# lhn0323/BEVFUSION-3D_object_detection

Hardware: AMD Instinct MI355X
Metric: nuScenes frames/sec (6-cam+LiDAR BEVFusion fwd+bwd) (higher is better)
Workload: dtype bf16; 1 GPU; full: BEVFusion camera+LiDAR (ResNet-50, LSS 6x256x704, hard voxelize 40k pts, sparse encoder, ConvFuser, SECOND/SECONDFPN, TransFusion head + Hungarian targets + focal/L1/gaussian-focal losses) fwd + bwd + clip + AdamW, bf16 autocast, fp32 index paths; global_batch=4, points_per_frame=40000, parallelism=independent frames per rank, execution=eager launches on 2 HIP queues (camera / BEV chain, LiDAR branch), view_transform_conv_dtype=bf16, head_fp32_conv=three bf16 products per multiply, fp32 accumulation (2^-16 relative per product), dense_weight_gradients=one grouped launch per tile shape at the end of the backward pass, backward_pass_thread=caller, trainable_params=37361053

## Files before the change

### bevfusion-3d_object_detection_amd/_lib.py

```python
import ctypes
import os

import torch

_HERE = os.path.dirname(os.path.abspath(__file__))
LIB_PATH = os.path.join(_HERE, "csrc", "libbevfusion_hip.so")

_c_int = ctypes.c_int
_c_vp = ctypes.c_void_p
_c_sz = ctypes.c_size_t

SIGNATURES = {
    "bfhip_abi_version": (_c_int, []),
    "bfhip_last_error": (ctypes.c_char_p, []),
    "bfhip_profile_enable": (None, [_c_int]),
    "bfhip_profile_read": (_c_int, [_c_int, _c_vp, _c_vp, _c_int]),
    "bfhip_bev_pool_fwd": (_c_int, [_c_vp] * 5 + [_c_int] * 7 + [_c_vp, _c_vp]),
    "bfhip_bev_pool_bwd": (_c_int, [_c_vp] * 5 + [_c_int] * 8 + [_c_vp, _c_vp]),
    "bfhip_dynamic_voxelize": (_c_int, [_c_vp, _c_vp, _c_int, _c_int, _c_vp, _c_vp, _c_vp]),
    "bfhip_hard_voxelize_workspace_bytes": (_c_sz, [_c_int, _c_int, _c_int]),
    "bfhip_hard_voxelize": (_c_int, [_c_vp, _c_int, _c_int, _c_vp, _c_vp, _c_vp, _c_vp, _c_vp,
                                     _c_int, _c_int, _c_vp, _c_sz, _c_vp, _c_vp]),
    "bfhip_bev_plan_workspace_bytes": (_c_sz, [ctypes.c_longlong, ctypes.c_longlong]),
    "bfhip_bev_plan": (_c_int, [_c_vp] * 7 + [_c_int] * 4 + [_c_vp] * 3 + [_c_vp] * 11 + [_c_int, _c_vp, _c_sz, _c_vp]),
# ... 80 lines not shown
    "bfhip_conv2d_wt_segment_bytes": (_c_int, []),
    "bfhip_conv2d_weight_transpose_batched": (_c_int, [_c_vp, _c_int, ctypes.c_longlong, _c_vp]),
    "bfhip_conv2d_launch_choice": (_c_int, [_c_int] * 12 + [_c_vp]),
    "bfhip_conv2d_wgrad_choice": (_c_int, [_c_int] * 10 + [_c_vp]),
    "bfhip_conv2d_wgrad_workspace_bytes": (_c_sz, [_c_int] * 7),
    "bfhip_conv2d_wgrad": (_c_int, [_c_vp, _c_int, _c_vp, _c_int, _c_vp] + [_c_int] * 11 + [_c_vp, _c_sz, _c_vp]),
    "bfhip_conv2d_wgrad_group_table_bytes": (_c_sz, [_c_int]),
    "bfhip_conv2d_wgrad_groupable": (_c_int, [_c_int] * 10),
    "bfhip_conv2d_wgrad_group_plan": (_c_int, [_c_vp, _c_int, _c_int, _c_vp, _c_sz, _c_vp]),
    "bfhip_conv2d_wgrad_group_launch": (_c_int, [_c_vp, _c_vp, _c_vp, _c_sz, _c_vp]),
    "bfhip_bn2d_fwd_partials": (_c_int, [_c_vp] * 4 + [ctypes.c_longlong, _c_int, _c_int, ctypes.c_float, ctypes.c_float, _c_int] +
                                [_c_vp] * 4 + [_c_vp, _c_int, _c_vp, _c_vp]),
    "bfhip_bn2d_fwd_partials_mask": (_c_int, [_c_vp] * 4 + [ctypes.c_longlong, _c_int, _c_int, ctypes.c_float, ctypes.c_float, _c_int] +
                                     [_c_vp] * 4 + [_c_vp, _c_int, _c_vp, _c_vp, _c_vp]),
    "bfhip_bn2d_bwd_mask": (_c_int, [_c_vp] * 5 + [ctypes.c_longlong, _c_int, _c_int] + [_c_vp] * 4 + [_c_vp, _c_sz, _c_vp]),
    "bfhip_adamw_segment_bytes": (_c_int, []),
    "bfhip_adamw_chunk_elems": (_c_int, []),
    "bfhip_adamw_step": (_c_int, [_c_vp, _c_vp, _c_vp, _c_int, _c_vp, _c_vp] + [ctypes.c_float] * 6 + [_c_vp]),
    "bfhip_adamw_step_groups": (_c_int, [_c_vp, _c_vp, _c_vp, _c_int, _c_vp, _c_vp, _c_vp, _c_vp, _c_int, ctypes.c_float, _c_vp]),
    "bfhip_query_losses": (_c_int, [_c_vp] * 7 + [_c_int] * 6 + [ctypes.c_float, ctypes.c_float] + [_c_vp] * 4),
    "bfhip_swin_attn_supported": (_c_int, [_c_int] * 7),
    "bfhip_swin_attn_parts": (_c_int, [_c_int] * 4),
    "bfhip_swin_attn_fwd": (_c_int, [_c_vp, ctypes.c_longlong, _c_vp] + [_c_int] * 5 + [ctypes.c_float, _c_vp, _c_vp, _c_vp]),
    "bfhip_swin_attn_bwd": (_c_int, [_c_vp, ctypes.c_longlong, _c_vp, _c_vp, _c_vp, _c_vp] + [_c_int] * 5 +
                            [ctypes.c_float, _c_vp, _c_vp, _c_int, _c_vp]),
    "bfhip_layernorm_supported": (_c_int, [ctypes.c_longlong, _c_int, _c_int, _c_int]),
    "bfhip_layernorm_parts": (_c_int, [ctypes.c_longlong, _c_int]),
    "bfhip_layernorm_fwd": (_c_int, [_c_vp, _c_vp, _c_vp, ctypes.c_longlong, _c_vp, _c_vp, ctypes.c_longlong, _c_int, ctypes.c_float] +
                            [_c_int] * 3 + [_c_vp] * 4),
    "bfhip_layernorm_bwd": (_c_int, [_c_vp] * 6 + [ctypes.c_longlong, ctypes.c_longlong] + [_c_int] * 4 + [_c_vp] * 3 + [_c_int] +
# ... 125 lines not shown
```

### bevfusion-3d_object_detection_amd/csrc/bn2d.hip

```cpp
#include <algorithm>
#include <map>
#include <mutex>

#include "common.h"

namespace bfhip {
namespace {

typedef unsigned short bf16_t;

template <typename T> struct Vec;
template <> struct Vec<float> {
  static constexpr int V = 4;
  static __device__ __forceinline__ void load(const float *p, float *o) {
    float4 v = *(const float4 *)p;
    o[0] = v.x; o[1] = v.y; o[2] = v.z; o[3] = v.w;
  }
  static __device__ __forceinline__ void store(float *p, const float *o) { *(float4 *)p = make_float4(o[0], o[1], o[2], o[3]); }
};
template <> struct Vec<bf16_t> {
  static constexpr int V = 8;
  static __device__ __forceinline__ void load(const bf16_t *p, float *o) {
    uint4 v = *(const uint4 *)p;
    const unsigned w[4] = {v.x, v.y, v.z, v.w};
// ... 99 lines not shown
    for (int g2 = 0; g2 < tr.ng; ++g2) {
      s += ld_agent(&tr.gp[((size_t)g2 * 2 + 0) * C + c]);
      s2 += ld_agent(&tr.gp[((size_t)g2 * 2 + 1) * C + c]);
    }
    fin(c, s, s2);
  }
}

struct FwdFin {
  long long M;
  const int *m_dev;
  int C;
  float eps, momentum;
  const float *gamma, *beta;
  float *stats, *running_mean, *running_var;
  __device__ __forceinline__ void operator()(int c, double s, double s2) const {
    long long Mv = M;
    if (m_dev) { long long mv = *m_dev; Mv = mv < 1 ? 1 : (mv < M ? mv : M); }
    double mean = s / (double)Mv;
    double var = s2 / (double)Mv - mean * mean;
    if (var < 0.0) var = 0.0;
    float invstd = (float)(1.0 / sqrt(var + (double)eps));
    float a = gamma[c] * invstd;
    stats[c] = (float)mean;
    stats[C + c] = invstd;
    stats[2 * C + c] = a;
    stats[3 * C + c] = beta[c] - (float)mean * a;
    if (running_mean) {
      double unbiased = Mv > 1 ? var * (double)Mv / (double)(Mv - 1) : var;
      running_mean[c] = (float)((1.0 - momentum) * running_mean[c] + momentum * mean);
      running_var[c] = (float)((1.0 - momentum) * running_var[c] + momentum * unbiased);
    }
  }
};

struct BwdFin {
  long long M;
  const int *m_dev;
  int C;
  const float *stats;
  float *dgb, *coef;
  __device__ __forceinline__ void operator()(int c, double s, double s2) const {
    long long Mv = M;
    if (m_dev) { long long mv = *m_dev; Mv = mv < 1 ? 1 : (mv < M ? mv : M); }
    const float mean = stats[c], invstd = stats[C + c], a = stats[2 * C + c];
    const float dbeta = (float)s, dgamma = (float)(s2 * (double)invstd);
    dgb[c] = dgamma;
    dgb[C + c] = dbeta;
    const float invM = (float)(1.0 / (double)Mv);
    const float c2 = -a * invstd * dgamma * invM;
    coef[c] = a;
    coef[C + c] = c2;
    coef[2 * C + c] = -a * dbeta * invM - c2 * mean;
  }
};

struct SumFin {
  int C;
  float *out;
  __device__ __forceinline__ void operator()(int c, double s, double) const { out[c] = (float)s; }
};

template <typename T>
__global__ __launch_bounds__(256) void bn2d_stats_kernel(const T *__restrict__ x, long long M, int C, Map mp,
                                                         float *__restrict__ partial, Tree tr, FwdFin fin) {
  constexpr int V = Vec<T>::V;
  __shared__ float sm[2 * 256 * V];
  const int t = threadIdx.x, cv = blockIdx.y * mp.Lb + t % mp.Lb, rl = t / mp.Lb;
// ... 60 lines not shown
  s = 0.0; s2 = 0.0;
  if (t < 8)
#pragma unroll
    for (int g = 0; g < 8; ++g) { s += sm[0][g * 8 + t]; s2 += sm[1][g * 8 + t]; }
}

template <typename Fin>
__global__ __launch_bounds__(kFinThreads) void bn2d_finalize_kernel(const float *__restrict__ partial, int nblk, Fin fin) {
  const int c = blockIdx.x * 8 + (threadIdx.x & 7);
  double s, s2;
  reduce_partials8(partial, nblk, fin.C, c, c < fin.C, s, s2);
  if (threadIdx.x >= 8 || c >= fin.C) return;
  fin(c, s, s2);
}

template <typename T, bool RES, bool RELU>
__global__ __launch_bounds__(256) void bn2d_apply_kernel(const T *__restrict__ x, const T *__restrict__ res,
                                                         const float *__restrict__ stats, long long M, int C, Map mp,
                                                         T *__restrict__ y, unsigned char *__restrict__ relu_mask) {
  constexpr int V = Vec<T>::V;
  const int t = threadIdx.x, cv = blockIdx.y * mp.Lb + t % mp.Lb, rl = t / mp.Lb;
  const bool live = rl < mp.R && cv * V < C;
  if (!live) return;
  float a[V], b[V];
#pragma unroll
  for (int j = 0; j < V; ++j) { a[j] = stats[2 * C + cv * V + j]; b[j] = stats[3 * C + cv * V + j]; }
  const long long r0 = (long long)blockIdx.x * mp.rpb, r1 = r0 + mp.rpb < M ? r0 + mp.rpb : M;
  const size_t col = (size_t)cv * V;
  long long r = r0 + rl;
  for (; r + mp.R < r1; r += 2LL * mp.R) {
    float v[2][V], q[2][V];
#pragma unroll
    for (int u = 0; u < 2; ++u) {
      Vec<T>::load(x + (size_t)(r + (long long)u * mp.R) * C + col, v[u]);
      if (RES) Vec<T>::load(res + (size_t)(r + (long long)u * mp.R) * C + col, q[u]);
    }
#pragma unroll
    for (int u = 0; u < 2; ++u) {
      unsigned bits = 0;
#pragma unroll
      for (int j = 0; j < V; ++j) {
        float o = v[u][j] * a[j] + b[j];
        if (RES) o += q[u][j];
        if (o > 0.f) bits |= 1u << j;
        v[u][j] = (RELU && !(o > 0.f)) ? 0.f : o;
      }
      Vec<T>::store(y + (size_t)(r + (long long)u * mp.R) * C + col, v[u]);
      if (V == 8 && relu_mask) relu_mask[(size_t)(r + (long long)u * mp.R) * (C >> 3) + cv] = (unsigned char)bits;
    }
  }
  for (; r < r1; r += mp.R) {
    float v[V], q[V];
    Vec<T>::load(x + (size_t)r * C + col, v);
    if (RES) Vec<T>::load(res + (size_t)r * C + col, q);
    unsigned bits = 0;
#pragma unroll
    for (int j = 0; j < V; ++j) {
      float o = v[j] * a[j] + b[j];
      if (RES) o += q[j];
      if (o > 0.f) bits |= 1u << j;
      v[j] = (RELU && !(o > 0.f)) ? 0.f : o;
    }
    Vec<T>::store(y + (size_t)r * C + col, v);
    if (V == 8 && relu_mask) relu_mask[(size_t)r * (C >> 3) + cv] = (unsigned char)bits;
  }
}

template <typename T, int MASK>
__device__ __forceinline__ void masked_grad(float *g, const float *xv, const float *yv, const float *a, const float *b) {
  constexpr int V = Vec<T>::V;
  const unsigned bits = MASK == 3 ? __float_as_uint(yv[0]) : 0u;
#pragma unroll
  for (int j = 0; j < V; ++j) {
    if (MASK == 1 && !(xv[j] * a[j] + b[j] > 0.f)) g[j] = 0.f;
    if (MASK == 2 && !(yv[j] > 0.f)) g[j] = 0.f;
    if (MASK == 3 && !((bits >> j) & 1u)) g[j] = 0.f;
  }
}

// ... 41 lines not shown
      float g[V], xv[V], yv[V];
      size_t off = (size_t)r * C + col;
      Vec<T>::load(dy + off, g);
      Vec<T>::load(x + off, xv);
      if (MASK == 2) Vec<T>::load(y + off, yv);
      if (MASK == 3) yv[0] = __uint_as_float(((const unsigned char *)y)[(size_t)r * (C >> 3) + cv]);
      masked_grad<T, MASK>(g, xv, yv, a, b);
#pragma unroll
      for (int j = 0; j < V; ++j) { s0[j] += g[j]; s1[j] += g[j] * (xv[j] - mean[j]); }
    }
  }
  combine_rows<V>(s0, s1, mp.Lb, mp.R, C, partial, sm);
  finish_in_last_block(partial, tr, C, blockIdx.y * mp.Lb * V, mp.Lb * V, fin);
}

template <typename T, int MASK, bool DRES>
__global__ __launch_bounds__(256) void bn2d_bwd_apply_kernel(const T *__restrict__ dy, const T *__restrict__ x,
                                                             const T *__restrict__ y,
                                                             const float *__restrict__ stats,
                                                             const float *__restrict__ coef, long long M, int C,
                                                             Map mp, T *__restrict__ dx, T *__restrict__ dres) {
  constexpr int V = Vec<T>::V;
  const int t = threadIdx.x, cv = blockIdx.y * mp.Lb + t % mp.Lb, rl = t / mp.Lb;
  const bool live = rl < mp.R && cv * V < C;
  if (!live) return;
  float a[V], b[V], c1[V], c2[V], c3[V];
#pragma unroll
  for (int j = 0; j < V; ++j) {
    a[j] = stats[2 * C + cv * V + j];
    b[j] = stats[3 * C + cv * V + j];
    c1[j] = coef[cv * V + j];
    c2[j] = coef[C + cv * V + j];
    c3[j] = coef[2 * C + cv * V + j];
  }
  const long long r0 = (long long)blockIdx.x * mp.rpb, r1 = r0 + mp.rpb < M ? r0 + mp.rpb : M;
  const size_t col = (size_t)cv * V;
  long long r = r0 + rl;
  for (; r + mp.R < r1; r += 2LL * mp.R) {
    float g[2][V], xv[2][V], yv[2][V];
#pragma unroll
    for (int u = 0; u < 2; ++u) {
      size_t off = (size_t)(r + (long long)u * mp.R) * C + col;
      Vec<T>::load(dy + off, g[u]);
      Vec<T>::load(x + off, xv[u]);
      if (MASK == 2) Vec<T>::load(y + off, yv[u]);
      if (MASK == 3) yv[u][0] = __uint_as_float(((const unsigned char *)y)[(size_t)(r + (long long)u * mp.R) * (C >> 3) + cv]);
    }
#pragma unroll
    for (int u = 0; u < 2; ++u) {
      size_t off = (size_t)(r + (long long)u * mp.R) * C + col;
      masked_grad<T, MASK>(g[u], xv[u], yv[u], a, b);
      if (DRES) Vec<T>::store(dres + off, g[u]);
#pragma unroll
      for (int j = 0; j < V; ++j) xv[u][j] = c1[j] * g[u][j] + c2[j] * xv[u][j] + c3[j];
      Vec<T>::store(dx + off, xv[u]);
    }
  }
  for (; r < r1; r += mp.R) {
    float g[V], xv[V], yv[V];
    size_t off = (size_t)r * C + col;
    Vec<T>::load(dy + off, g);
    Vec<T>::load(x + off, xv);
    if (MASK == 2) Vec<T>::load(y + off, yv);
    if (MASK == 3) yv[0] = __uint_as_float(((const unsigned char *)y)[(size_t)r * (C >> 3) + cv]);
    masked_grad<T, MASK>(g, xv, yv, a, b);
    if (DRES) Vec<T>::store(dres + off, g);
#pragma unroll
    for (int j = 0; j < V; ++j) xv[j] = c1[j] * g[j] + c2[j] * xv[j] + c3[j];
    Vec<T>::store(dx + off, xv);
  }
}

inline int elem_size(int dtype) { return dtype == 1 ? 2 : 4; }

inline bool shape_ok(long long M, int C, int dtype) {
  const int V = 16 / elem_size(dtype);
  return M > 0 && C >= V && C % V == 0 && C <= 65536;
}

inline Map make_map(long long M, int C, int dtype, dim3 *grid) {
  const int es = elem_size(dtype), V = 16 / es, L = C / V;
  Map mp;
  mp.Lb = L < 32 ? L : 32;
  mp.R = 256 / mp.Lb;
  const int CT = (L + mp.Lb - 1) / mp.Lb;
  long long S = 1024;
  S = std::min(S, (M + 4LL * mp.R - 1) / (4LL * mp.R));
  S = std::min(S, (long long)std::max(1, 2048 / CT));
  S = std::min(S, std::max(1LL, M * es / 128));
  S = std::max(S, 1LL);
  long long rpb = ((M + S - 1) / S + mp.R - 1) / mp.R * mp.R;
  S = (M + rpb - 1) / rpb;
  mp.rpb = (int)rpb;
  *grid = dim3((unsigned)S, (unsigned)CT);
  return mp;
}

template <typename T>
int run_fwd(const void *x, const void *res, const float *stats, long long M, int C, Map mp, dim3 grid, int relu, void *y,
            hipStream_t s, unsigned char *relu_mask = nullptr) {
#define BFHIP_BN2D_APPLY(RES, RELU)                                                                             \
  hipLaunchKernelGGL((bn2d_apply_kernel<T, RES, RELU>), grid, dim3(256), 0, s, (const T *)x, (const T *)res, \
                     stats, M, C, mp, (T *)y, (RES && RELU) ? relu_mask : (unsigned char *)nullptr)
  if (res) { if (relu) BFHIP_BN2D_APPLY(true, true); else BFHIP_BN2D_APPLY(true, false); }
  else { if (relu) BFHIP_BN2D_APPLY(false, true); else BFHIP_BN2D_APPLY(false, false); }
#undef BFHIP_BN2D_APPLY
  return 0;
}

template <typename T, int MASK>
void run_bwd(const void *dy, const void *x, const void *y, const float *stats, long long M, int C, Map mp, dim3 grid,
             float *partial, float *coef, Tree tr, BwdFin fin, void *dx, void *dres, hipStream_t s) {
  hipLaunchKernelGGL((bn2d_bwd_reduce_kernel<T, MASK>), grid, dim3(256), 0, s, (const T *)dy, (const T *)x,
                     (const T *)y, stats, M, C, mp, partial, tr, fin);
  if (!tr.cnt) hipLaunchKernelGGL(bn2d_finalize_kernel<BwdFin>, dim3(ceil_div(C, 8)), dim3(kFinThreads), 0, s, partial, tr.nblk, fin);
  if (dres)
    hipLaunchKernelGGL((bn2d_bwd_apply_kernel<T, MASK, true>), grid, dim3(256), 0, s, (const T *)dy, (const T *)x,
                       (const T *)y, stats, coef, M, C, mp, (T *)dx, (T *)dres);
  else
    hipLaunchKernelGGL((bn2d_bwd_apply_kernel<T, MASK, false>), grid, dim3(256), 0, s, (const T *)dy,
                       (const T *)x, (const T *)y, stats, coef, M, C, mp, (T *)dx, (T *)nullptr);
}

constexpr int kSlabInts = 16384;
constexpr int kSlabs = 32;

inline bool fold_enabled() {
  static const bool on = [] { const char *e = env_str("BFHIP_BN2D_FOLD"); return e && e[0] == '1'; }();
  return on;
}

int *arrival_counters(hipStream_t stream) {
  static std::mutex mu;
  static std::map<int, int *> pool;
  static std::map<std::pair<int, hipStream_t>, int> slot;
  static std::map<int, int> used;
  int dev = 0;
  if (hipGetDevice(&dev) != hipSuccess) return nullptr;
  std::lock_guard<std::mutex> lock(mu);
  auto it = pool.find(dev);
  if (it == pool.end()) {
    int *p = nullptr;
    const size_t bytes = (size_t)kSlabs * kSlabInts * sizeof(int);
    if (hipMalloc((void **)&p, bytes) != hipSuccess || hipMemset(p, 0, bytes) != hipSuccess) {
      set_error("bn2d: cannot allocate the arrival counters (first call on a device must be outside a stream capture)");
// ... 2 lines not shown
    it = pool.emplace(dev, p).first;
  }
  auto key = std::make_pair(dev, stream);
  auto st = slot.find(key);
  if (st == slot.end()) {
    if (used[dev] >= kSlabs) { set_error("bn2d: more than %d streams per device in use", kSlabs); return nullptr; }
    st = slot.emplace(key, used[dev]++).first;
  }
  return it->second + (size_t)st->second * kSlabInts;
}

struct Plan {
  Map mp;
  dim3 grid;
  int nblk, ng;
  float *partial, *coef;
  double *gp;
};

inline size_t plan_bytes(long long M, int C, int dtype, Plan *pl, void *workspace) {
  pl->mp = make_map(M, C, dtype, &pl->grid);
  pl->nblk = (int)pl->grid.x;
  pl->ng = (pl->nblk + kGroup - 1) / kGroup;
  size_t off = 0;
  pl->partial = (float *)((char *)workspace + off); off += align_up((size_t)pl->nblk * 2 * C * sizeof(float), 256);
  pl->coef = (float *)((char *)workspace + off); off += align_up((size_t)3 * C * sizeof(float), 256);
  pl->gp = (double *)((char *)workspace + off); off += align_up((size_t)pl->ng * 2 * C * sizeof(double), 256);
  return off;
}

}
}

using namespace bfhip;

BFHIP_EXPORT int bfhip_bn2d_supported(long long M, int C, int dtype) {
  return (dtype == 0 || dtype == 1) && shape_ok(M, C, dtype) ? 1 : 0;
}

BFHIP_EXPORT size_t bfhip_bn2d_workspace_bytes(long long M, int C, int dtype) {
  if (!bfhip_bn2d_supported(M, C, dtype)) return 0;
  Plan pl;
  return plan_bytes(M, C, dtype, &pl, nullptr);
}

BFHIP_EXPORT int bfhip_colsum(const void *x, long long M, int C, int dtype, float *out, void *workspace, size_t workspace_bytes,
                              void *stream_) {
  hipStream_t s = (hipStream_t)stream_;
  BFHIP_REQUIRE(bfhip_bn2d_supported(M, C, dtype), "colsum: unsupported shape M=%lld C=%d dtype=%d", M, C, dtype);
  BFHIP_REQUIRE(x && out && ((uintptr_t)x % 16) == 0, "colsum: null or misaligned pointer");
  if (!workspace || workspace_bytes < bfhip_bn2d_workspace_bytes(M, C, dtype)) { set_error("colsum: workspace too small"); return BFHIP_E_WORKSPACE; }
  Plan pl;
  plan_bytes(M, C, dtype, &pl, workspace);
  Tree tr{nullptr, pl.gp, pl.nblk, pl.ng};
  FwdFin none{};
  if (dtype == 1)
    hipLaunchKernelGGL(bn2d_stats_kernel<bf16_t>, pl.grid, dim3(256), 0, s, (const bf16_t *)x, M, C, pl.mp, pl.partial, tr, none);
  else
    hipLaunchKernelGGL(bn2d_stats_kernel<float>, pl.grid, dim3(256), 0, s, (const float *)x, M, C, pl.mp, pl.partial, tr, none);
  hipLaunchKernelGGL(bn2d_finalize_kernel<SumFin>, dim3(ceil_div(C, 8)), dim3(kFinThreads), 0, s, pl.partial, pl.nblk, SumFin{C, out});
  return check_launch("colsum");
}

BFHIP_EXPORT int bfhip_bn2d_fwd(const void *x, const void *residual, const float *gamma, const float *beta,
                                long long M, int C, int dtype, float eps, float momentum, int relu,
                                float *running_mean, float *running_var, float *stats, void *y, const int32_t *m_dev,
                                void *workspace, size_t workspace_bytes, void *stream_) {
  hipStream_t s = (hipStream_t)stream_;
// ... 3 lines not shown
                "bn2d_fwd: tensors must be 16-byte aligned");
  if (!workspace || workspace_bytes < bfhip_bn2d_workspace_bytes(M, C, dtype)) { set_error("bn2d_fwd: workspace too small"); return BFHIP_E_WORKSPACE; }
  Plan pl;
  plan_bytes(M, C, dtype, &pl, workspace);
  int *cnt = fold_enabled() ? arrival_counters(s) : nullptr;
  if (!cnt && fold_enabled()) return BFHIP_E_LAUNCH;
  BFHIP_REQUIRE((long long)pl.grid.y * (1 + pl.ng) <= kSlabInts, "bn2d_fwd: too many column tiles");
  Tree tr{cnt, pl.gp, pl.nblk, pl.ng};
  FwdFin fin{M, m_dev, C, eps, momentum, gamma, beta, stats, running_mean, running_var};
  ProfScope ps;
  prof_begin(BFHIP_OP_BN2D_FWD, s, &ps);
  if (dtype == 1)
    hipLaunchKernelGGL(bn2d_stats_kernel<bf16_t>, pl.grid, dim3(256), 0, s, (const bf16_t *)x, M, C, pl.mp, pl.partial, tr, fin);
  else
    hipLaunchKernelGGL(bn2d_stats_kernel<float>, pl.grid, dim3(256), 0, s, (const float *)x, M, C, pl.mp, pl.partial, tr, fin);
  if (!cnt) hipLaunchKernelGGL(bn2d_finalize_kernel<FwdFin>, dim3(ceil_div(C, 8)), dim3(kFinThreads), 0, s, pl.partial, pl.nblk, fin);
  if (dtype == 1) run_fwd<bf16_t>(x, residual, stats, M, C, pl.mp, pl.grid, relu, y, s);
  else run_fwd<float>(x, residual, stats, M, C, pl.mp, pl.grid, relu, y, s);
  prof_end(&ps);
  return check_launch("bn2d_fwd");
}

static int bn2d_fwd_partials_impl(const void *x, const void *residual, const float *gamma, const float *beta, long long M, int C,
                                  int dtype, float eps, float momentum, int relu, float *running_mean, float *running_var,
                                  float *stats, void *y, const float *partial, int nblk, const int32_t *m_dev,
                                  unsigned char *relu_mask, void *stream_) {
  hipStream_t s = (hipStream_t)stream_;
  BFHIP_REQUIRE(!relu_mask || (dtype == 1 && relu && residual), "bn2d_fwd_partials: a ReLU bit mask needs bf16 + residual + ReLU");
  BFHIP_REQUIRE(bfhip_bn2d_supported(M, C, dtype), "bn2d_fwd_partials: unsupported shape M=%lld C=%d dtype=%d", M, C, dtype);
  BFHIP_REQUIRE(x && gamma && beta && stats && y && partial && nblk > 0, "bn2d_fwd_partials: null pointer");
  BFHIP_REQUIRE(((uintptr_t)x % 16) == 0 && ((uintptr_t)y % 16) == 0 && ((uintptr_t)residual % 16) == 0,
                "bn2d_fwd_partials: tensors must be 16-byte aligned");
  dim3 grid;
  Map mp = make_map(M, C, dtype, &grid);
  FwdFin fin{M, m_dev, C, eps, momentum, gamma, beta, stats, running_mean, running_var};
  ProfScope ps;
  prof_begin(BFHIP_OP_BN2D_FWD, s, &ps);
  hipLaunchKernelGGL(bn2d_finalize_kernel<FwdFin>, dim3(ceil_div(C, 8)), dim3(kFinThreads), 0, s, partial, nblk, fin);
  if (dtype == 1) run_fwd<bf16_t>(x, residual, stats, M, C, mp, grid, relu, y, s, relu_mask);
  else run_fwd<float>(x, residual, stats, M, C, mp, grid, relu, y, s);
  prof_end(&ps);
  return check_launch("bn2d_fwd_partials");
}

BFHIP_EXPORT int bfhip_bn2d_fwd_partials(const void *x, const void *residual, const float *gamma, const float *beta,
                                         long long M, int C, int dtype, float eps, float momentum, int relu,
                                         float *running_mean, float *running_var, float *stats, void *y,
                                         const float *partial, int nblk, const int32_t *m_dev, void *stream_) {
  return bn2d_fwd_partials_impl(x, residual, gamma, beta, M, C, dtype, eps, momentum, relu, running_mean, running_var, stats, y,
                                partial, nblk, m_dev, nullptr, stream_);
}

BFHIP_EXPORT int bfhip_bn2d_fwd_partials_mask(const void *x, const void *residual, const float *gamma, const float *beta,
                                              long long M, int C, int dtype, float eps, float momentum, int relu,
                                              float *running_mean, float *running_var, float *stats, void *y,
// ... 13 lines not shown
  BFHIP_REQUIRE(bfhip_bn2d_supported(M, C, dtype), "bn2d_bwd: unsupported shape M=%lld C=%d dtype=%d", M, C, dtype);
  BFHIP_REQUIRE(dy && x && stats && gamma && dx && dgb, "bn2d_bwd: null pointer");
  BFHIP_REQUIRE(((uintptr_t)dy % 16) == 0 && ((uintptr_t)x % 16) == 0 && ((uintptr_t)dx % 16) == 0 &&
                    ((uintptr_t)y % 16) == 0 && ((uintptr_t)dres % 16) == 0, "bn2d_bwd: tensors must be 16-byte aligned");
  if (!workspace || workspace_bytes < bfhip_bn2d_workspace_bytes(M, C, dtype)) { set_error("bn2d_bwd: workspace too small"); return BFHIP_E_WORKSPACE; }
  Plan pl;
  plan_bytes(M, C, dtype, &pl, workspace);
  int *cnt = fold_enabled() ? arrival_counters(s) : nullptr;
  if (!cnt && fold_enabled()) return BFHIP_E_LAUNCH;
  BFHIP_REQUIRE((long long)pl.grid.y * (1 + pl.ng) <= kSlabInts, "bn2d_bwd: too many column tiles");
  Tree tr{cnt, pl.gp, pl.nblk, pl.ng};
  BwdFin fin{M, m_dev, C, stats, dgb, pl.coef};
  const int mask = !relu ? 0 : (relu_mask ? 3 : (y ? 2 : 1));
  ProfScope ps;
  prof_begin(BFHIP_OP_BN2D_BWD, s, &ps);
#define BFHIP_BN2D_BWD(T, MASK) run_bwd<T, MASK>(dy, x, y, stats, M, C, pl.mp, pl.grid, pl.partial, pl.coef, tr, fin, dx, dres, s)
  if (dtype == 1) {
    if (mask == 0) BFHIP_BN2D_BWD(bf16_t, 0);
    else if (mask == 1) BFHIP_BN2D_BWD(bf16_t, 1);
    else if (mask == 3) BFHIP_BN2D_BWD(bf16_t, 3);
    else BFHIP_BN2D_BWD(bf16_t, 2);
  } else {
    if (mask == 0) BFHIP_BN2D_BWD(float, 0);
    else if (mask == 1) BFHIP_BN2D_BWD(float, 1);
    else BFHIP_BN2D_BWD(float, 2);
  }
#undef BFHIP_BN2D_BWD
  prof_end(&ps);
  return check_launch("bn2d_bwd");
}

// ... 14 lines not shown
```

### include/bevfusion_hip.h

```cpp
#ifndef BEVFUSION_HIP_H_
#define BEVFUSION_HIP_H_

#include <stddef.h>
#include <stdint.h>

#ifdef __cplusplus
extern "C" {
#endif

#define BFHIP_OK 0
#define BFHIP_E_INVALID (-1)
#define BFHIP_E_WORKSPACE (-2)
#define BFHIP_E_LAUNCH (-3)

#define BFHIP_REDUCE_SUM 0
#define BFHIP_REDUCE_MEAN 1
#define BFHIP_REDUCE_MAX 2

#define BFHIP_OP_BEV_POOL_FWD 0
#define BFHIP_OP_BEV_POOL_BWD 1
#define BFHIP_OP_HARD_VOXELIZE 2
#define BFHIP_OP_DYNAMIC_VOXELIZE 3
#define BFHIP_OP_LIFT_SPLAT_FWD 4
#define BFHIP_OP_LIFT_SPLAT_BWD 5
// ... 236 lines not shown
size_t bfhip_conv2d_wgrad_group_table_bytes(int n_layers);
int bfhip_conv2d_wgrad_groupable(int N, int H, int W, int Cin, int Cout, int KH, int KW, int stride, int pad, int dil);
int bfhip_conv2d_wgrad_group_plan(const void *layers, int n_layers, int target_steps, void *table_host, size_t table_bytes,
                                  size_t *slab_bytes);
int bfhip_conv2d_wgrad_group_launch(const void *table_host, const void *table_dev, void *slab, size_t slab_bytes, void *stream);
int bfhip_bn2d_fwd_partials(const void *x, const void *residual, const float *gamma, const float *beta, long long M, int C,
                            int dtype, float eps, float momentum, int relu, float *running_mean, float *running_var,
                            float *stats, void *y, const float *partial, int nblk, const int32_t *m_dev, void *stream);
int bfhip_bn2d_fwd_partials_mask(const void *x, const void *residual, const float *gamma, const float *beta, long long M, int C,
                                 int dtype, float eps, float momentum, int relu, float *running_mean, float *running_var,
                                 float *stats, void *y, const float *partial, int nblk, const int32_t *m_dev,
                                 unsigned char *relu_mask, void *stream);
int bfhip_bn2d_bwd_mask(const void *dy, const void *x, const unsigned char *relu_mask, const float *stats, const float *gamma,
                        long long M, int C, int dtype, void *dx, void *dres, float *dgb, const int32_t *m_dev, void *workspace,
                        size_t workspace_bytes, void *stream);

int bfhip_adamw_segment_bytes(void);
int bfhip_adamw_chunk_elems(void);
int bfhip_adamw_step(const void *segs_dev, const int64_t *grad_ptrs_dev, const int32_t *chunks_dev, int n_chunks,
                     float *partial_dev, float *scalars_dev, float lr, float beta1, float beta2, float eps,
                     float weight_decay, float max_norm, void *stream);
int bfhip_adamw_step_groups(const void *segs_dev, const int64_t *grad_ptrs_dev, const int32_t *chunks_dev, int n_chunks,
                            float *partial_dev, float *scalars_dev, float *groups_dev, const float *groups_host, int n_groups,
                            float max_norm, void *stream);

int bfhip_swin_attn_supported(int B, int Hp, int Wp, int heads, int window, int head_dim, int shift);
int bfhip_swin_attn_parts(int B, int Hp, int Wp, int heads);
int bfhip_swin_attn_fwd(const void *qkv, long long qkv_pitch, const float *bias, int B, int Hp, int Wp, int heads, int shift,
                        float scale, void *out, float *lse, void *stream);
int bfhip_swin_attn_bwd(const void *qkv, long long qkv_pitch, const float *bias, const void *out, const void *dout,
// ... 35 lines not shown
```

Baseline: 155.3 frames/s.

## Fold BN2d finalize into apply kernels via per-block partial reduction

Adds a self-finalizing path to the BN2d forward and backward apply kernels. Each block sums the per-block partials for its channel tile in shared memory and computes scale/shift or backward coefficients itself, so the separate finalize launch and its global round trip are dropped. The first tile rows are prefetched before the reduction to hide its latency. The cost is redundant partial reduction in every row block and more shared memory, and choose_chain picks this path by shape.

Result: no change. 155.9 frames/s (median of 4 runs) (+0.4%).

```diff
diff --git a/bevfusion-3d_object_detection_amd/_lib.py b/bevfusion-3d_object_detection_amd/_lib.py
--- a/bevfusion-3d_object_detection_amd/_lib.py
+++ b/bevfusion-3d_object_detection_amd/_lib.py
@@ -118,6 +118,7 @@
     "bfhip_bn2d_fwd_partials_mask": (_c_int, [_c_vp] * 4 + [ctypes.c_longlong, _c_int, _c_int, ctypes.c_float, ctypes.c_float, _c_int] +
                                      [_c_vp] * 4 + [_c_vp, _c_int, _c_vp, _c_vp, _c_vp]),
     "bfhip_bn2d_bwd_mask": (_c_int, [_c_vp] * 5 + [ctypes.c_longlong, _c_int, _c_int] + [_c_vp] * 4 + [_c_vp, _c_sz, _c_vp]),
+    "bfhip_bn2d_chain_choice": (_c_int, [ctypes.c_longlong, _c_int, _c_int, _c_int, _c_int, _c_vp]),
     "bfhip_adamw_segment_bytes": (_c_int, []),
     "bfhip_adamw_chunk_elems": (_c_int, []),
     "bfhip_adamw_step": (_c_int, [_c_vp, _c_vp, _c_vp, _c_int, _c_vp, _c_vp] + [ctypes.c_float] * 6 + [_c_vp]),
diff --git a/bevfusion-3d_object_detection_amd/csrc/bn2d.hip b/bevfusion-3d_object_detection_amd/csrc/bn2d.hip
--- a/bevfusion-3d_object_detection_amd/csrc/bn2d.hip
+++ b/bevfusion-3d_object_detection_amd/csrc/bn2d.hip
@@ -137,24 +137,31 @@
   float eps, momentum;
   const float *gamma, *beta;
   float *stats, *running_mean, *running_var;
-  __device__ __forceinline__ void operator()(int c, double s, double s2) const {
-    long long Mv = M;
-    if (m_dev) { long long mv = *m_dev; Mv = mv < 1 ? 1 : (mv < M ? mv : M); }
-    double mean = s / (double)Mv;
-    double var = s2 / (double)Mv - mean * mean;
-    if (var < 0.0) var = 0.0;
-    float invstd = (float)(1.0 / sqrt(var + (double)eps));
-    float a = gamma[c] * invstd;
-    stats[c] = (float)mean;
-    stats[C + c] = invstd;
-    stats[2 * C + c] = a;
-    stats[3 * C + c] = beta[c] - (float)mean * a;
+  struct Val { double mean, var; long long Mv; float invstd, a, b; };
+  __device__ __forceinline__ Val values(int c, double s, double s2) const {
+    Val v;
+    v.Mv = M;
+    if (m_dev) { long long mv = *m_dev; v.Mv = mv < 1 ? 1 : (mv < M ? mv : M); }
+    v.mean = s / (double)v.Mv;
+    v.var = s2 / (double)v.Mv - v.mean * v.mean;
+    if (v.var < 0.0) v.var = 0.0;
+    v.invstd = (float)(1.0 / sqrt(v.var + (double)eps));
+    v.a = gamma[c] * v.invstd;
+    v.b = beta[c] - (float)v.mean * v.a;
+    return v;
+  }
+  __device__ __forceinline__ void store(int c, const Val &v) const {
+    stats[c] = (float)v.mean;
+    stats[C + c] = v.invstd;
+    stats[2 * C + c] = v.a;
+    stats[3 * C + c] = v.b;
     if (running_mean) {
-      double unbiased = Mv > 1 ? var * (double)Mv / (double)(Mv - 1) : var;
-      running_mean[c] = (float)((1.0 - momentum) * running_mean[c] + momentum * mean);
+      double unbiased = v.Mv > 1 ? v.var * (double)v.Mv / (double)(v.Mv - 1) : v.var;
+      running_mean[c] = (float)((1.0 - momentum) * running_mean[c] + momentum * v.mean);
       running_var[c] = (float)((1.0 - momentum) * running_var[c] + momentum * unbiased);
     }
   }
+  __device__ __forceinline__ void operator()(int c, double s, double s2) const { store(c, values(c, s, s2)); }
 };
 
 struct BwdFin {
@@ -163,18 +170,30 @@
   int C;
   const float *stats;
   float *dgb, *coef;
-  __device__ __forceinline__ void operator()(int c, double s, double s2) const {
+  struct Val { float dgamma, dbeta, c1, c2, c3; };
+  __device__ __forceinline__ Val values(int c, double s, double s2) const {
     long long Mv = M;
     if (m_dev) { long long mv = *m_dev; Mv = mv < 1 ? 1 : (mv < M ? mv : M); }
     const float mean = stats[c], invstd = stats[C + c], a = stats[2 * C + c];
-    const float dbeta = (float)s, dgamma = (float)(s2 * (double)invstd);
-    dgb[c] = dgamma;
-    dgb[C + c] = dbeta;
+    Val v;
+    v.dbeta = (float)s;
+    v.dgamma = (float)(s2 * (double)invstd);
     const float invM = (float)(1.0 / (double)Mv);
-    const float c2 = -a * invstd * dgamma * invM;
-    coef[c] = a;
-    coef[C + c] = c2;
-    coef[2 * C + c] = -a * dbeta * invM - c2 * mean;
+    v.c1 = a;
+    v.c2 = -a * invstd * v.dgamma * invM;
+    v.c3 = -a * v.dbeta * invM - v.c2 * mean;
+    return v;
+  }
+  __device__ __forceinline__ void store_dgb(int c, const Val &v) const {
+    dgb[c] = v.dgamma;
+    dgb[C + c] = v.dbeta;
+  }
+  __device__ __forceinline__ void operator()(int c, double s, double s2) const {
+    const Val v = values(c, s, s2);
+    store_dgb(c, v);
+    coef[c] = v.c1;
+    coef[C + c] = v.c2;
+    coef[2 * C + c] = v.c3;
   }
 };
 
@@ -265,45 +284,99 @@
   fin(c, s, s2);
 }
 
-template <typename T, bool RES, bool RELU>
+constexpr int kSfRows = 10;
+constexpr int kSfMaxLanes = 32;
+constexpr int kSfMaxCh = 128;
+constexpr int kSfBudget = 9216;
+constexpr int kSfMaxRowsCap = 160;
+
+struct SelfFin {
+  double part[2 * 1024];
+  double tot[2 * kSfMaxCh];
+  float co[5 * kSfMaxCh];
+};
+
+__device__ __forceinline__ void sum_tile_partials(const float *__restrict__ partial, int nblk, int C, int c0, int nch,
+                                                  SelfFin &sf) {
+  const int t = threadIdx.x, q = nch >> 2;
+  const int lanes = 256 / q < kSfMaxLanes ? 256 / q : kSfMaxLanes;
+  const int cq = t % q, kl = t / q;
+  if (kl < lanes) {
+    double a[4] = {0.0, 0.0, 0.0, 0.0}, b[4] = {0.0, 0.0, 0.0, 0.0};
+    if (c0 + 4 * cq < C) {
+      const float *p = partial + c0 + 4 * cq;
+      for (int k0 = kl; k0 < nblk; k0 += kSfRows * lanes) {
+        float4 v0[kSfRows], v1[kSfRows];
+#pragma unroll
+        for (int u = 0; u < kSfRows; ++u) {
+          const int k = k0 + u * lanes, kc = k < nblk ? k : nblk - 1;
+          v0[u] = *(const float4 *)(p + ((size_t)kc * 2 + 0) * C);
+          v1[u] = *(const float4 *)(p + ((size_t)kc * 2 + 1) * C);
+        }
+#pragma unroll
+        for (int u = 0; u < kSfRows; ++u)
+          if (k0 + u * lanes < nblk) {
+            a[0] += (double)v0[u].x; a[1] += (double)v0[u].y; a[2] += (double)v0[u].z; a[3] += (double)v0[u].w;
+            b[0] += (double)v1[u].x; b[1] += (double)v1[u].y; b[2] += (double)v1[u].z; b[3] += (double)v1[u].w;
+          }
+      }
+    }
+#pragma unroll
+    for (int j = 0; j < 4; ++j) {
+      sf.part[(0 * lanes + kl) * nch + 4 * cq + j] = a[j];
+      sf.part[(1 * lanes + kl) * nch + 4 * cq + j] = b[j];
+    }
+  }
+  __syncthreads();
+  if (t < 2 * nch) {
+    const int sidx = t / nch, ch = t % nch;
+    double acc = 0.0;
+    for (int l = 0; l < lanes; ++l) acc += sf.part[(sidx * lanes + l) * nch + ch];
+    sf.tot[t] = acc;
+  }
+  __syncthreads();
+}
+
+template <typename T, bool RES, bool RELU, bool SELF>
 __global__ __launch_bounds__(256) void bn2d_apply_kernel(const T *__restrict__ x, const T *__restrict__ res,
                                                          const float *__restrict__ stats, long long M, int C, Map mp,
-                                                         T *__restrict__ y, unsigned char *__restrict__ relu_mask) {
+                                                         T *__restrict__ y, unsigned char *__restrict__ relu_mask,
+                                                         const float *__restrict__ partial, int nblk, FwdFin fin) {
   constexpr int V = Vec<T>::V;
   const int t = threadIdx.x, cv = blockIdx.y * mp.Lb + t % mp.Lb, rl = t / mp.Lb;
   const bool live = rl < mp.R && cv * V < C;
-  if (!live) return;
+  if (!SELF && !live) return;
+  const long long r0 = (long long)blockIdx.x * mp.rpb, r1 = r0 + mp.rpb < M ? r0 + mp.rpb : M;
+  const size_t col = live ? (size_t)cv * V : 0;
+  long long r = r0 + rl;
   float a[V], b[V];
-#pragma unroll
-  for (int j = 0; j < V; ++j) { a[j] = stats[2 * C + cv * V + j]; b[j] = stats[3 * C + cv * V + j]; }
-  const long long r0 = (long long)blockIdx.x * mp.rpb, r1 = r0 + mp.rpb < M ? r0 + mp.rpb : M;
-  const size_t col = (size_t)cv * V;
-  long long r = r0 + rl;
-  for (; r + mp.R < r1; r += 2LL * mp.R) {
-    float v[2][V], q[2][V];
+  float v0[2][V], q0[2][V];
+  if (SELF) {
 #pragma unroll
     for (int u = 0; u < 2; ++u) {
-      Vec<T>::load(x + (size_t)(r + (long long)u * mp.R) * C + col, v[u]);
-      if (RES) Vec<T>::load(res + (size_t)(r + (long long)u * mp.R) * C + col, q[u]);
-    }
-#pragma unroll
-    for (int u = 0; u < 2; ++u) {
-      unsigned bits = 0;
-#pragma unroll
-      for (int j = 0; j < V; ++j) {
-        float o = v[u][j] * a[j] + b[j];
-        if (RES) o += q[u][j];
-        if (o > 0.f) bits |= 1u << j;
-        v[u][j] = (RELU && !(o > 0.f)) ? 0.f : o;
-      }
-      Vec<T>::store(y + (size_t)(r + (long long)u * mp.R) * C + col, v[u]);
-      if (V == 8 && relu_mask) relu_mask[(size_t)(r + (long long)u * mp.R) * (C >> 3) + cv] = (unsigned char)bits;
-    }
-  }
-  for (; r < r1; r += mp.R) {
-    float v[V], q[V];
-    Vec<T>::load(x + (size_t)r * C + col, v);
-    if (RES) Vec<T>::load(res + (size_t)r * C + col, q);
+      long long rr = r + (long long)u * mp.R;
+      rr = rr < M ? rr : M - 1;
+      Vec<T>::load(x + (size_t)rr * C + col, v0[u]);
+      if (RES) Vec<T>::load(res + (size_t)rr * C + col, q0[u]);
+    }
+    __shared__ SelfFin sf;
+    const int nch = mp.Lb * V, c0 = blockIdx.y * nch;
+    sum_tile_partials(partial, nblk, C, c0, nch, sf);
+    if (t < nch && c0 + t < C) {
+      const FwdFin::Val w = fin.values(c0 + t, sf.tot[t], sf.tot[nch + t]);
+      sf.co[t] = w.a;
+      sf.co[kSfMaxCh + t] = w.b;
+      if (blockIdx.x == 0) fin.store(c0 + t, w);
+    }
+    __syncthreads();
+    if (!live) return;
+#pragma unroll
+    for (int j = 0; j < V; ++j) { a[j] = sf.co[(t % mp.Lb) * V + j]; b[j] = sf.co[kSfMaxCh + (t % mp.Lb) * V + j]; }
+  } else {
+#pragma unroll
+    for (int j = 0; j < V; ++j) { a[j] = stats[2 * C + cv * V + j]; b[j] = stats[3 * C + cv * V + j]; }
+  }
+  auto row = [&](long long rr, float *v, const float *q) {
     unsigned bits = 0;
 #pragma unroll
     for (int j = 0; j < V; ++j) {
@@ -312,8 +385,34 @@
       if (o > 0.f) bits |= 1u << j;
       v[j] = (RELU && !(o > 0.f)) ? 0.f : o;
     }
-    Vec<T>::store(y + (size_t)r * C + col, v);
-    if (V == 8 && relu_mask) relu_mask[(size_t)r * (C >> 3) + cv] = (unsigned char)bits;
+    Vec<T>::store(y + (size_t)rr * C + col, v);
+    if (V == 8 && relu_mask) relu_mask[(size_t)rr * (C >> 3) + cv] = (unsigned char)bits;
+  };
+  if (SELF) {
+    if (r + mp.R < r1) {
+      row(r, v0[0], q0[0]);
+      row(r + mp.R, v0[1], q0[1]);
+      r += 2LL * mp.R;
+    } else if (r < r1) {
+      row(r, v0[0], q0[0]);
+      r += mp.R;
+    }
+  }
+  for (; r + mp.R < r1; r += 2LL * mp.R) {
+    float v[2][V], q[2][V];
+#pragma unroll
+    for (int u = 0; u < 2; ++u) {
+      Vec<T>::load(x + (size_t)(r + (long long)u * mp.R) * C + col, v[u]);
+      if (RES) Vec<T>::load(res + (size_t)(r + (long long)u * mp.R) * C + col, q[u]);
+    }
+#pragma unroll
+    for (int u = 0; u < 2; ++u) row(r + (long long)u * mp.R, v[u], q[u]);
+  }
+  for (; r < r1; r += mp.R) {
+    float v[V], q[V];
+    Vec<T>::load(x + (size_t)r * C + col, v);
+    if (RES) Vec<T>::load(res + (size_t)r * C + col, q);
+    row(r, v, q);
   }
 }
 
@@ -385,60 +484,97 @@
   finish_in_last_block(partial, tr, C, blockIdx.y * mp.Lb * V, mp.Lb * V, fin);
 }
 
-template <typename T, int MASK, bool DRES>
+template <typename T, int MASK, bool DRES, bool SELF>
 __global__ __launch_bounds__(256) void bn2d_bwd_apply_kernel(const T *__restrict__ dy, const T *__restrict__ x,
                                                              const T *__restrict__ y,
                                                              const float *__restrict__ stats,
                                                              const float *__restrict__ coef, long long M, int C,
-                                                             Map mp, T *__restrict__ dx, T *__restrict__ dres) {
+                                                             Map mp, T *__restrict__ dx, T *__restrict__ dres,
+                                                             const float *__restrict__ partial, int nblk, BwdFin fin) {
   constexpr int V = Vec<T>::V;
   const int t = threadIdx.x, cv = blockIdx.y * mp.Lb + t % mp.Lb, rl = t / mp.Lb;
   const bool live = rl < mp.R && cv * V < C;
-  if (!live) return;
+  if (!SELF && !live) return;
+  const long long r0 = (long long)blockIdx.x * mp.rpb, r1 = r0 + mp.rpb < M ? r0 + mp.rpb : M;
+  const size_t col = live ? (size_t)cv * V : 0;
+  const int cvm = live ? cv : 0;
+  long long r = r0 + rl;
+  auto load_row = [&](long long rr, float *g, float *xv, float *yv) {
+    const size_t off = (size_t)rr * C + col;
+    Vec<T>::load(dy + off, g);
+    Vec<T>::load(x + off, xv);
+    if (MASK == 2) Vec<T>::load(y + off, yv);
+    if (MASK == 3) yv[0] = __uint_as_float(((const unsigned char *)y)[(size_t)rr * (C >> 3) + cvm]);
+  };
   float a[V], b[V], c1[V], c2[V], c3[V];
+  float g0[2][V], x0[2][V], y0[2][V];
+  if (SELF) {
+#pragma unroll
+    for (int u = 0; u < 2; ++u) {
+      long long rr = r + (long long)u * mp.R;
+      load_row(rr < M ? rr : M - 1, g0[u], x0[u], y0[u]);
+    }
+    __shared__ SelfFin sf;
+    const int nch = mp.Lb * V, c0 = blockIdx.y * nch;
+    sum_tile_partials(partial, nblk, C, c0, nch, sf);
+    if (t < nch && c0 + t < C) {
+      const BwdFin::Val w = fin.values(c0 + t, sf.tot[t], sf.tot[nch + t]);
+      sf.co[t] = w.c1;
+      sf.co[kSfMaxCh + t] = w.c2;
+      sf.co[2 * kSfMaxCh + t] = w.c3;
+      if (blockIdx.x == 0) fin.store_dgb(c0 + t, w);
+    }
+    __syncthreads();
+    if (!live) return;
+#pragma unroll
+    for (int j = 0; j < V; ++j) {
+      const int cl = (t % mp.Lb) * V + j;
+      c1[j] = sf.co[cl];
+      c2[j] = sf.co[kSfMaxCh + cl];
+      c3[j] = sf.co[2 * kSfMaxCh + cl];
+    }
+  } else {
+#pragma unroll
+    for (int j = 0; j < V; ++j) {
+      c1[j] = coef[cv * V + j];
+      c2[j] = coef[C + cv * V + j];
+      c3[j] = coef[2 * C + cv * V + j];
+    }
+  }
 #pragma unroll
   for (int j = 0; j < V; ++j) {
     a[j] = stats[2 * C + cv * V + j];
     b[j] = stats[3 * C + cv * V + j];
-    c1[j] = coef[cv * V + j];
-    c2[j] = coef[C + cv * V + j];
-    c3[j] = coef[2 * C + cv * V + j];
-  }
-  const long long r0 = (long long)blockIdx.x * mp.rpb, r1 = r0 + mp.rpb < M ? r0 + mp.rpb : M;
-  const size_t col = (size_t)cv * V;
-  long long r = r0 + rl;
+  }
+  auto row = [&](long long rr, float *g, float *xv, const float *yv) {
+    const size_t off = (size_t)rr * C + col;
+    masked_grad<T, MASK>(g, xv, yv, a, b);
+    if (DRES) Vec<T>::store(dres + off, g);
+#pragma unroll
+    for (int j = 0; j < V; ++j) xv[j] = c1[j] * g[j] + c2[j] * xv[j] + c3[j];
+    Vec<T>::store(dx + off, xv);
+  };
+  if (SELF) {
+    if (r + mp.R < r1) {
+      row(r, g0[0], x0[0], y0[0]);
+      row(r + mp.R, g0[1], x0[1], y0[1]);
+      r += 2LL * mp.R;
+    } else if (r < r1) {
+      row(r, g0[0], x0[0], y0[0]);
+      r += mp.R;
+    }
+  }
   for (; r + mp.R < r1; r += 2LL * mp.R) {
     float g[2][V], xv[2][V], yv[2][V];
 #pragma unroll
-    for (int u = 0; u < 2; ++u) {
-      size_t off = (size_t)(r + (long long)u * mp.R) * C + col;
-      Vec<T>::load(dy + off, g[u]);
-      Vec<T>::load(x + off, xv[u]);
-      if (MASK == 2) Vec<T>::load(y + off, yv[u]);
-      if (MASK == 3) yv[u][0] = __uint_as_float(((const unsigned char *)y)[(size_t)(r + (long long)u * mp.R) * (C >> 3) + cv]);
-    }
-#pragma unroll
-    for (int u = 0; u < 2; ++u) {
-      size_t off = (size_t)(r + (long long)u * mp.R) * C + col;
-      masked_grad<T, MASK>(g[u], xv[u], yv[u], a, b);
-      if (DRES) Vec<T>::store(dres + off, g[u]);
-#pragma unroll
-      for (int j = 0; j < V; ++j) xv[u][j] = c1[j] * g[u][j] + c2[j] * xv[u][j] + c3[j];
-      Vec<T>::store(dx + off, xv[u]);
-    }
+    for (int u = 0; u < 2; ++u) load_row(r + (long long)u * mp.R, g[u], xv[u], yv[u]);
+#pragma unroll
+    for (int u = 0; u < 2; ++u) row(r + (long long)u * mp.R, g[u], xv[u], yv[u]);
   }
   for (; r < r1; r += mp.R) {
     float g[V], xv[V], yv[V];
-    size_t off = (size_t)r * C + col;
-    Vec<T>::load(dy + off, g);
-    Vec<T>::load(x + off, xv);
-    if (MASK == 2) Vec<T>::load(y + off, yv);
-    if (MASK == 3) yv[0] = __uint_as_float(((const unsigned char *)y)[(size_t)r * (C >> 3) + cv]);
-    masked_grad<T, MASK>(g, xv, yv, a, b);
-    if (DRES) Vec<T>::store(dres + off, g);
-#pragma unroll
-    for (int j = 0; j < V; ++j) xv[j] = c1[j] * g[j] + c2[j] * xv[j] + c3[j];
-    Vec<T>::store(dx + off, xv);
+    load_row(r, g, xv, yv);
+    row(r, g, xv, yv);
   }
 }
 
@@ -467,39 +603,97 @@
   return mp;
 }
 
-template <typename T>
-int run_fwd(const void *x, const void *res, const float *stats, long long M, int C, Map mp, dim3 grid, int relu, void *y,
-            hipStream_t s, unsigned char *relu_mask = nullptr) {
-#define BFHIP_BN2D_APPLY(RES, RELU)                                                                             \
-  hipLaunchKernelGGL((bn2d_apply_kernel<T, RES, RELU>), grid, dim3(256), 0, s, (const T *)x, (const T *)res, \
-                     stats, M, C, mp, (T *)y, (RES && RELU) ? relu_mask : (unsigned char *)nullptr)
-  if (res) { if (relu) BFHIP_BN2D_APPLY(true, true); else BFHIP_BN2D_APPLY(true, false); }
-  else { if (relu) BFHIP_BN2D_APPLY(false, true); else BFHIP_BN2D_APPLY(false, false); }
-#undef BFHIP_BN2D_APPLY
-  return 0;
-}
-
-template <typename T, int MASK>
-void run_bwd(const void *dy, const void *x, const void *y, const float *stats, long long M, int C, Map mp, dim3 grid,
-             float *partial, float *coef, Tree tr, BwdFin fin, void *dx, void *dres, hipStream_t s) {
-  hipLaunchKernelGGL((bn2d_bwd_reduce_kernel<T, MASK>), grid, dim3(256), 0, s, (const T *)dy, (const T *)x,
-                     (const T *)y, stats, M, C, mp, partial, tr, fin);
-  if (!tr.cnt) hipLaunchKernelGGL(bn2d_finalize_kernel<BwdFin>, dim3(ceil_div(C, 8)), dim3(kFinThreads), 0, s, partial, tr.nblk, fin);
-  if (dres)
-    hipLaunchKernelGGL((bn2d_bwd_apply_kernel<T, MASK, true>), grid, dim3(256), 0, s, (const T *)dy, (const T *)x,
-                       (const T *)y, stats, coef, M, C, mp, (T *)dx, (T *)dres);
-  else
-    hipLaunchKernelGGL((bn2d_bwd_apply_kernel<T, MASK, false>), grid, dim3(256), 0, s, (const T *)dy,
-                       (const T *)x, (const T *)y, stats, coef, M, C, mp, (T *)dx, (T *)nullptr);
-}
-
-constexpr int kSlabInts = 16384;
-constexpr int kSlabs = 32;
-
 inline bool fold_enabled() {
   static const bool on = [] { const char *e = env_str("BFHIP_BN2D_FOLD"); return e && e[0] == '1'; }();
   return on;
 }
+
+inline int self_fin_mode() {
+  static const int mode = [] {
+    if (fold_enabled()) return 0;
+    const char *e = env_str("BFHIP_BN2D_SELF_FIN");
+    if (!e || !e[0]) return 1;
+    return e[0] == '0' ? 0 : (e[0] == '2' ? 2 : 1);
+  }();
+  return mode;
+}
+
+struct Chain {
+  bool self;
+  Map mp;
+  dim3 grid;
+  int rows;
+};
+
+inline bool make_map_self(long long M, int C, int dtype, int partial_rows, Chain *ch) {
+  const int es = elem_size(dtype), V = 16 / es, L = C / V;
+  Map mp;
+  mp.Lb = L < 8 ? L : 8;
+  mp.R = 256 / mp.Lb;
+  const int nch = mp.Lb * V, CT = (L + mp.Lb - 1) / mp.Lb;
+  const int max_rows = std::min(kSfMaxRowsCap, kSfBudget / nch);
+  if (CT > 65535 || partial_rows > max_rows) return false;
+  long long S = (M + 4LL * mp.R - 1) / (4LL * mp.R);
+  if (partial_rows > 0) S = std::min(S, (long long)std::max(1, 512 / CT));
+  else S = std::min(S, (long long)max_rows);
+  S = std::min(S, std::max(1LL, M * es / 128));
+  S = std::max(S, 1LL);
+  long long rpb = ((M + S - 1) / S + mp.R - 1) / mp.R * mp.R;
+  S = (M + rpb - 1) / rpb;
+  mp.rpb = (int)rpb;
+  ch->self = true;
+  ch->mp = mp;
+  ch->grid = dim3((unsigned)S, (unsigned)CT);
+  ch->rows = partial_rows > 0 ? partial_rows : (int)S;
+  return true;
+}
+
+constexpr int kSfRuleMaxIters = 8;
+constexpr int kSfRuleMaxBlocks = 640;
+inline bool self_rule(const Chain &ch, int partial_rows) {
+  return partial_rows > 0 && ch.mp.rpb / ch.mp.R <= kSfRuleMaxIters && (long long)ch.grid.x * ch.grid.y <= kSfRuleMaxBlocks;
+}
+
+inline Chain choose_chain(long long M, int C, int dtype, int partial_rows) {
+  Chain ch;
+  const int mode = self_fin_mode();
+  if (mode != 0 && make_map_self(M, C, dtype, partial_rows, &ch) && (mode == 2 || self_rule(ch, partial_rows))) return ch;
+  ch.self = false;
+  ch.mp = make_map(M, C, dtype, &ch.grid);
+  ch.rows = partial_rows > 0 ? partial_rows : (int)ch.grid.x;
+  return ch;
+}
+
+template <typename T>
+int run_fwd(const void *x, const void *res, const float *stats, long long M, int C, Map mp, dim3 grid, int relu, void *y,
+            hipStream_t s, unsigned char *relu_mask, bool self, const float *partial, int nblk, const FwdFin &fin) {
+#define BFHIP_BN2D_APPLY(RES, RELU, SELF)                                                                             \
+  hipLaunchKernelGGL((bn2d_apply_kernel<T, RES, RELU, SELF>), grid, dim3(256), 0, s, (const T *)x, (const T *)res, \
+                     stats, M, C, mp, (T *)y, (RES && RELU) ? relu_mask : (unsigned char *)nullptr, partial, nblk, fin)
+#define BFHIP_BN2D_APPLY2(RES, RELU) do { if (self) BFHIP_BN2D_APPLY(RES, RELU, true); else BFHIP_BN2D_APPLY(RES, RELU, false); } while (0)
+  if (res) { if (relu) BFHIP_BN2D_APPLY2(true, true); else BFHIP_BN2D_APPLY2(true, false); }
+  else { if (relu) BFHIP_BN2D_APPLY2(false, true); else BFHIP_BN2D_APPLY2(false, false); }
+#undef BFHIP_BN2D_APPLY2
+#undef BFHIP_BN2D_APPLY
+  return 0;
+}
+
+template <typename T, int MASK>
+void run_bwd(const void *dy, const void *x, const void *y, const float *stats, long long M, int C, Map mp, dim3 grid,
+             float *partial, float *coef, Tree tr, BwdFin fin, void *dx, void *dres, hipStream_t s, bool self) {
+  hipLaunchKernelGGL((bn2d_bwd_reduce_kernel<T, MASK>), grid, dim3(256), 0, s, (const T *)dy, (const T *)x,
+                     (const T *)y, stats, M, C, mp, partial, tr, fin);
+  if (!tr.cnt && !self) hipLaunchKernelGGL(bn2d_finalize_kernel<BwdFin>, dim3(ceil_div(C, 8)), dim3(kFinThreads), 0, s, partial, tr.nblk, fin);
+#define BFHIP_BN2D_BWD_APPLY(DRES, SELF)                                                                                  \
+  hipLaunchKernelGGL((bn2d_bwd_apply_kernel<T, MASK, DRES, SELF>), grid, dim3(256), 0, s, (const T *)dy, (const T *)x, \
+                     (const T *)y, stats, coef, M, C, mp, (T *)dx, (T *)(DRES ? dres : nullptr), partial, tr.nblk, fin)
+  if (dres) { if (self) BFHIP_BN2D_BWD_APPLY(true, true); else BFHIP_BN2D_BWD_APPLY(true, false); }
+  else { if (self) BFHIP_BN2D_BWD_APPLY(false, true); else BFHIP_BN2D_BWD_APPLY(false, false); }
+#undef BFHIP_BN2D_BWD_APPLY
+}
+
+constexpr int kSlabInts = 16384;
+constexpr int kSlabs = 32;
 
 int *arrival_counters(hipStream_t stream) {
   static std::mutex mu;
@@ -532,18 +726,29 @@
   Map mp;
   dim3 grid;
   int nblk, ng;
+  bool self;
   float *partial, *coef;
   double *gp;
 };
 
-inline size_t plan_bytes(long long M, int C, int dtype, Plan *pl, void *workspace) {
-  pl->mp = make_map(M, C, dtype, &pl->grid);
+inline size_t plan_bytes(long long M, int C, int dtype, Plan *pl, void *workspace, bool allow_self = true) {
+  Chain ch = allow_self ? choose_chain(M, C, dtype, 0) : Chain{};
+  if (!allow_self) { ch.self = false; ch.mp = make_map(M, C, dtype, &ch.grid); }
+  pl->mp = ch.mp;
+  pl->grid = ch.grid;
+  pl->self = ch.self;
   pl->nblk = (int)pl->grid.x;
   pl->ng = (pl->nblk + kGroup - 1) / kGroup;
+  dim3 g0;
+  make_map(M, C, dtype, &g0);
+  Chain cs;
+  int rows = (int)g0.x;
+  if (make_map_self(M, C, dtype, 0, &cs)) rows = std::max(rows, cs.rows);
+  const int ng = (rows + kGroup - 1) / kGroup;
   size_t off = 0;
-  pl->partial = (float *)((char *)workspace + off); off += align_up((size_t)pl->nblk * 2 * C * sizeof(float), 256);
+  pl->partial = (float *)((char *)workspace + off); off += align_up((size_t)rows * 2 * C * sizeof(float), 256);
   pl->coef = (float *)((char *)workspace + off); off += align_up((size_t)3 * C * sizeof(float), 256);
-  pl->gp = (double *)((char *)workspace + off); off += align_up((size_t)pl->ng * 2 * C * sizeof(double), 256);
+  pl->gp = (double *)((char *)workspace + off); off += align_up((size_t)ng * 2 * C * sizeof(double), 256);
   return off;
 }
 
@@ -560,6 +765,20 @@
   if (!bfhip_bn2d_supported(M, C, dtype)) return 0;
   Plan pl;
   return plan_bytes(M, C, dtype, &pl, nullptr);
+}
+
+BFHIP_EXPORT int bfhip_bn2d_chain_choice(long long M, int C, int dtype, int partial_rows, int dir, int32_t *out) {
+  BFHIP_REQUIRE(out, "bn2d_chain_choice: null pointer");
+  BFHIP_REQUIRE(bfhip_bn2d_supported(M, C, dtype), "bn2d_chain_choice: unsupported shape M=%lld C=%d dtype=%d", M, C, dtype);
+  BFHIP_REQUIRE((dir == 0 || dir == 1) && partial_rows >= 0 && !(dir == 1 && partial_rows > 0),
+                "bn2d_chain_choice: dir is 0 | 1, partial rows belong to the forward");
+  const Chain ch = choose_chain(M, C, dtype, partial_rows);
+  const int fin_launch = (ch.self || (partial_rows == 0 && fold_enabled())) ? 0 : 1;
+  out[0] = (partial_rows > 0 ? 1 : 2) + fin_launch;
+  out[1] = ch.self ? 1 : 0;
+  out[2] = (int32_t)ch.grid.x;
+  out[3] = ch.mp.Lb;
+  return 0;
 }
 
 BFHIP_EXPORT int bfhip_colsum(const void *x, long long M, int C, int dtype, float *out, void *workspace, size_t workspace_bytes,
@@ -569,7 +788,7 @@
   BFHIP_REQUIRE(x && out && ((uintptr_t)x % 16) == 0, "colsum: null or misaligned pointer");
   if (!workspace || workspace_bytes < bfhip_bn2d_workspace_bytes(M, C, dtype)) { set_error("colsum: workspace too small"); return BFHIP_E_WORKSPACE; }
   Plan pl;
-  plan_bytes(M, C, dtype, &pl, workspace);
+  plan_bytes(M, C, dtype, &pl, workspace, false);
   Tree tr{nullptr, pl.gp, pl.nblk, pl.ng};
   FwdFin none{};
   if (dtype == 1)
@@ -603,9 +822,9 @@
     hipLaunchKernelGGL(bn2d_stats_kernel<bf16_t>, pl.grid, dim3(256), 0, s, (const bf16_t *)x, M, C, pl.mp, pl.partial, tr, fin);
   else
     hipLaunchKernelGGL(bn2d_stats_kernel<float>, pl.grid, dim3(256), 0, s, (const float *)x, M, C, pl.mp, pl.partial, tr, fin);
-  if (!cnt) hipLaunchKernelGGL(bn2d_finalize_kernel<FwdFin>, dim3(ceil_div(C, 8)), dim3(kFinThreads), 0, s, pl.partial, pl.nblk, fin);
-  if (dtype == 1) run_fwd<bf16_t>(x, residual, stats, M, C, pl.mp, pl.grid, relu, y, s);
-  else run_fwd<float>(x, residual, stats, M, C, pl.mp, pl.grid, relu, y, s);
+  if (!cnt && !pl.self) hipLaunchKernelGGL(bn2d_finalize_kernel<FwdFin>, dim3(ceil_div(C, 8)), dim3(kFinThreads), 0, s, pl.partial, pl.nblk, fin);
+  if (dtype == 1) run_fwd<bf16_t>(x, residual, stats, M, C, pl.mp, pl.grid, relu, y, s, nullptr, pl.self, pl.partial, pl.nblk, fin);
+  else run_fwd<float>(x, residual, stats, M, C, pl.mp, pl.grid, relu, y, s, nullptr, pl.self, pl.partial, pl.nblk, fin);
   prof_end(&ps);
   return check_launch("bn2d_fwd");
 }
@@ -620,14 +839,17 @@
   BFHIP_REQUIRE(x && gamma && beta && stats && y && partial && nblk > 0, "bn2d_fwd_partials: null pointer");
   BFHIP_REQUIRE(((uintptr_t)x % 16) == 0 && ((uintptr_t)y % 16) == 0 && ((uintptr_t)residual % 16) == 0,
                 "bn2d_fwd_partials: tensors must be 16-byte aligned");
-  dim3 grid;
-  Map mp = make_map(M, C, dtype, &grid);
+  Chain ch = choose_chain(M, C, dtype, nblk);
+  if (ch.self && ((uintptr_t)partial % 16) != 0) {
+    ch.self = false;
+    ch.mp = make_map(M, C, dtype, &ch.grid);
+  }
   FwdFin fin{M, m_dev, C, eps, momentum, gamma, beta, stats, running_mean, running_var};
   ProfScope ps;
   prof_begin(BFHIP_OP_BN2D_FWD, s, &ps);
-  hipLaunchKernelGGL(bn2d_finalize_kernel<FwdFin>, dim3(ceil_div(C, 8)), dim3(kFinThreads), 0, s, partial, nblk, fin);
-  if (dtype == 1) run_fwd<bf16_t>(x, residual, stats, M, C, mp, grid, relu, y, s, relu_mask);
-  else run_fwd<float>(x, residual, stats, M, C, mp, grid, relu, y, s);
+  if (!ch.self) hipLaunchKernelGGL(bn2d_finalize_kernel<FwdFin>, dim3(ceil_div(C, 8)), dim3(kFinThreads), 0, s, partial, nblk, fin);
+  if (dtype == 1) run_fwd<bf16_t>(x, residual, stats, M, C, ch.mp, ch.grid, relu, y, s, relu_mask, ch.self, partial, nblk, fin);
+  else run_fwd<float>(x, residual, stats, M, C, ch.mp, ch.grid, relu, y, s, nullptr, ch.self, partial, nblk, fin);
   prof_end(&ps);
   return check_launch("bn2d_fwd_partials");
 }
@@ -671,7 +893,7 @@
   const int mask = !relu ? 0 : (relu_mask ? 3 : (y ? 2 : 1));
   ProfScope ps;
   prof_begin(BFHIP_OP_BN2D_BWD, s, &ps);
-#define BFHIP_BN2D_BWD(T, MASK) run_bwd<T, MASK>(dy, x, y, stats, M, C, pl.mp, pl.grid, pl.partial, pl.coef, tr, fin, dx, dres, s)
+#define BFHIP_BN2D_BWD(T, MASK) run_bwd<T, MASK>(dy, x, y, stats, M, C, pl.mp, pl.grid, pl.partial, pl.coef, tr, fin, dx, dres, s, pl.self)
   if (dtype == 1) {
     if (mask == 0) BFHIP_BN2D_BWD(bf16_t, 0);
     else if (mask == 1) BFHIP_BN2D_BWD(bf16_t, 1);
diff --git a/include/bevfusion_hip.h b/include/bevfusion_hip.h
--- a/include/bevfusion_hip.h
+++ b/include/bevfusion_hip.h
@@ -274,6 +274,7 @@
 int bfhip_bn2d_bwd_mask(const void *dy, const void *x, const unsigned char *relu_mask, const float *stats, const float *gamma,
                         long long M, int C, int dtype, void *dx, void *dres, float *dgb, const int32_t *m_dev, void *workspace,
                         size_t workspace_bytes, void *stream);
+int bfhip_bn2d_chain_choice(long long M, int C, int dtype, int partial_rows, int dir, int32_t *out_host);
 
 int bfhip_adamw_segment_bytes(void);
 int bfhip_adamw_chunk_elems(void);
```
